# fpthink/EPC-Net

Hardware: AMD Instinct MI355X
Metric: point-clouds/sec (4096 pts) descriptor extraction (higher is better)
Workload: dtype f16x3; 1 GPU; epc-net inference, batch 64x4096x3 fp32 per GPU, NetVLAD K=64, 256-D output (BASELINE.json configs[1]); num_points=4096, precision=EPC_PRECISION_F32 (include/epcnet.h), weights=seeded random init of the architecture (no checkpoint payloads exist), parallelism=independent clouds sharded over 1 GPU(s), no data-path collective

## Files before the change

### epc-net_amd/csrc/head.hip

```cpp
#include "common.h"



template <int GROUPS>
__global__ __launch_bounds__(256) void vlad_fold_kernel(const float* __restrict__ V, const float* __restrict__ colss,
                                                        float* __restrict__ U) {
    constexpr int FPG = 1024 / GROUPS;
    __shared__ float cn[64];
    __shared__ float gsum[64];
    const int slab = blockIdx.x, cloud = blockIdx.y;
    const int k = threadIdx.x & 63, r = threadIdx.x >> 6;
    if (r == 0) {
        float t = 0.f;
#pragma unroll
        for (int g = 0; g < 32; ++g) t += colss[((size_t)cloud * 32 + g) * 64 + k];
        const float inv = 1.0f / sqrtf(fmaxf(t, 1e-12f));
        cn[k] = inv;
        gsum[k] = t * inv * inv;
    }
    __syncthreads();
    float tot = 0.f;
#pragma unroll
    for (int q = 0; q < 64; ++q) tot += gsum[q];
    const float sc = cn[k] * (1.0f / sqrtf(fmaxf(tot, 1e-12f)));
    const float* v = V + (size_t)cloud * 1024 * 64;
    float* uo = U + (size_t)cloud * FPG * 64;
#pragma unroll
    for (int m = 0; m < 4; ++m) {
        const int fi = 16 * slab + r + 4 * m;
        float u = 0.f;
#pragma unroll
        for (int g = 0; g < GROUPS; ++g) u += v[(size_t)(g * FPG + fi) * 64 + k] * sc;
        uo[(size_t)fi * 64 + k] = u;
    }
}

#define HSL 128
__global__ __launch_bounds__(64) void hidden_gemm_kernel(const float* __restrict__ U, const float* __restrict__ H,
                                                         int rows, int kh, float* __restrict__ Yp) {
    const int lane = threadIdx.x, j = lane & 31, h = lane >> 5;
    const int nb = blockIdx.x * 32;
    const int slice = blockIdx.y;
    const int m0 = blockIdx.z * 64;
    const int k0 = slice * HSL;
    f32x16 acc[2];
#pragma unroll
    for (int r = 0; r < 16; ++r) acc[0][r] = acc[1][r] = 0.f;
    const int r0 = m0 + j, r1 = m0 + 32 + j;
    const float* a0p = U + (size_t)min(r0, rows - 1) * kh + k0 + 4 * h;
    const float* a1p = U + (size_t)min(r1, rows - 1) * kh + k0 + 4 * h;
    const float z0 = r0 < rows ? 1.f : 0.f, z1 = r1 < rows ? 1.f : 0.f;
    const float* bp = H + (size_t)(k0 + 4 * h) * 256 + nb + j;
#pragma unroll 8
    for (int q = 0; q < HSL / 8; ++q) {
        const float4 a0 = *reinterpret_cast<const float4*>(a0p + 8 * q);
        const float4 a1 = *reinterpret_cast<const float4*>(a1p + 8 * q);
        const float b0 = bp[(size_t)(8 * q + 0) * 256], b1 = bp[(size_t)(8 * q + 1) * 256];
        const float b2 = bp[(size_t)(8 * q + 2) * 256], b3 = bp[(size_t)(8 * q + 3) * 256];
        acc[0] = mfma32(a0.x * z0, b0, acc[0]);
        acc[1] = mfma32(a1.x * z1, b0, acc[1]);
        acc[0] = mfma32(a0.y * z0, b1, acc[0]);
        acc[1] = mfma32(a1.y * z1, b1, acc[1]);
        acc[0] = mfma32(a0.z * z0, b2, acc[0]);
        acc[1] = mfma32(a1.z * z1, b2, acc[1]);
        acc[0] = mfma32(a0.w * z0, b3, acc[0]);
        acc[1] = mfma32(a1.w * z1, b3, acc[1]);
    }
#pragma unroll
    for (int t = 0; t < 2; ++t)
#pragma unroll
        for (int r = 0; r < 16; ++r) {
            const int row = m0 + 32 * t + mfma_row(r, h);
            if (row < rows) Yp[((size_t)slice * rows + row) * 256 + nb + j] = acc[t][r];
        }
}

__global__ __launch_bounds__(1024) void head_finish_kernel(const float* __restrict__ Yp, int slices, int rows,
                                                           const float* __restrict__ hp, int groups,
                                                           const int32_t* __restrict__ status,
                                                           float* __restrict__ out) {
    __shared__ float part_y[4][256];
    __shared__ float v[256];
    __shared__ float red[4];
    const int cloud = blockIdx.x, c = threadIdx.x & 255, part = threadIdx.x >> 8;
    const float* bn_s = hp;
    const float* bn_t = hp + 256;
    const float* Wg = hp + 512;
    const float* g_s = Wg + 65536;
    const float* g_t = g_s + 256;
    float y = 0.f;
    int s = part;
    for (; s + 28 < slices; s += 32) {
        float t[8];
#pragma unroll
        for (int u = 0; u < 8; ++u) t[u] = Yp[((size_t)(s + 4 * u) * rows + cloud) * 256 + c];
#pragma unroll
        for (int u = 0; u < 8; ++u) y += t[u];
    }
    for (; s < slices; s += 4) y += Yp[((size_t)s * rows + cloud) * 256 + c];
    part_y[part][c] = y;
    __syncthreads();
    const float val = ((part_y[0][c] + part_y[1][c]) + (part_y[2][c] + part_y[3][c])) * bn_s[c] + (float)groups * bn_t[c];
    if (part == 0) v[c] = val;
    __syncthreads();
    float g = 0.f;
#pragma unroll 16
    for (int k = 64 * part; k < 64 * part + 64; ++k) g += v[k] * Wg[k * 256 + c];
    part_y[part][c] = g;
    __syncthreads();
    g = (part_y[0][c] + part_y[1][c]) + (part_y[2][c] + part_y[3][c]);
    g = g * g_s[c] + g_t[c];
    const float o = val * (1.0f / (1.0f + expf(-g)));
    float ss = o * o;
#pragma unroll
    for (int off = 32; off >= 1; off >>= 1) ss += __shfl_xor(ss, off);
    if (part == 0 && (c & 63) == 0) red[c >> 6] = ss;
    __syncthreads();
    const float tot = (red[0] + red[1]) + (red[2] + red[3]);
    const bool poisoned = status && status[cloud] != 0;
    if (part == 0) out[(size_t)cloud * 256 + c] = poisoned ? __int_as_float(0x7fc00000) : o * (1.0f / sqrtf(fmaxf(tot, 1e-12f)));
}

__global__ __launch_bounds__(1024) void fc_head_kernel(const float* __restrict__ pooled,
                                                       const float* __restrict__ pack,
                                                       const int32_t* __restrict__ status, float* __restrict__ out) {
    __shared__ float m[1024];
    __shared__ float part_y[4][256];
    __shared__ float red[4];
    const int cloud = blockIdx.x, c = threadIdx.x & 255, part = threadIdx.x >> 8;
    m[threadIdx.x] = pooled[(size_t)cloud * 1024 + threadIdx.x];
    __syncthreads();
    float y = 0.f;
#pragma unroll 16
    for (int k = 256 * part; k < 256 * part + 256; ++k) y += m[k] * pack[k * 256 + c];
    part_y[part][c] = y;
    __syncthreads();
    y = fmaxf(((part_y[0][c] + part_y[1][c]) + (part_y[2][c] + part_y[3][c])) + pack[1024 * 256 + c], 0.f);
    float ss = y * y;
#pragma unroll
    for (int off = 32; off >= 1; off >>= 1) ss += __shfl_xor(ss, off);
    if (part == 0 && (c & 63) == 0) red[c >> 6] = ss;
    __syncthreads();
    const float tot = (red[0] + red[1]) + (red[2] + red[3]);
    const bool poisoned = status && status[cloud] != 0;
    if (part == 0) out[(size_t)cloud * 256 + c] = poisoned ? __int_as_float(0x7fc00000) : y * (1.0f / sqrtf(fmaxf(tot, 1e-12f)));
}

static inline size_t align_up(size_t v, size_t a) { return (v + a - 1) / a * a; }

extern "C" size_t epc_vlad_head_workspace_bytes(int num_clouds, int groups) {
    if (num_clouds <= 0 || groups <= 0 || 64 % groups) return 0;
    const size_t kh = 65536 / groups;
    const size_t u = align_up((size_t)num_clouds * kh * sizeof(float), 256);
    const size_t yp = align_up((kh / HSL) * (size_t)num_clouds * 256 * sizeof(float), 256);
    return u + yp;
}

extern "C" int epc_vlad_head_fwd(const float* V, const float* colss, const void* packed_head, int groups,
                                 int num_clouds, float* out, const int32_t* status, void* workspace,
                                 size_t workspace_bytes, void* stream) {
    EPC_CHECK_ARG(V && colss && packed_head && out && workspace, "null pointer");
    EPC_CHECK_ARG(groups > 0 && 64 % groups == 0, "GROUPS must divide 64");
    EPC_CHECK_ARG(num_clouds >= 0, "bad shape");
    if (num_clouds == 0) return EPC_OK;
    if (workspace_bytes < epc_vlad_head_workspace_bytes(num_clouds, groups)) {
        epc_set_error("epc_vlad_head_fwd: workspace too small");
        return EPC_ENOMEM;
    }
    const int kh = 65536 / groups;
    const float* hp = (const float*)packed_head;
    const float* Hw = hp + 65536;
    const float* tail = Hw + (size_t)kh * 256;
    char* wsp = (char*)workspace;
    float* U = (float*)wsp;
    wsp += align_up((size_t)num_clouds * kh * sizeof(float), 256);
    float* Yp = (float*)wsp;
    hipStream_t st = (hipStream_t)stream;
    EPC_CHECK_ARG(num_clouds <= 65535, "too many clouds per call");
    switch (groups) {
#define EPC_VF(G)                                                                                                  \
    case G:                                                                                                        \
        hipLaunchKernelGGL(vlad_fold_kernel<G>, dim3(1024 / G / 16, num_clouds), dim3(256), 0, st, V, colss, U);   \
        break;
        EPC_VF(1) EPC_VF(2) EPC_VF(4) EPC_VF(8) EPC_VF(16)
#undef EPC_VF
        default:
            epc_set_error("epc_vlad_head_fwd: GROUPS must be one of 1,2,4,8,16");
            return EPC_EINVAL;
    }
    EPC_CHECK_LAUNCH();
    const int slices = kh / HSL;
    hipLaunchKernelGGL(hidden_gemm_kernel, dim3(8, slices, (num_clouds + 63) / 64), dim3(64), 0, st, U, Hw,
                       num_clouds, kh, Yp);
    EPC_CHECK_LAUNCH();
    hipLaunchKernelGGL(head_finish_kernel, dim3(num_clouds), dim3(1024), 0, st, Yp, slices, num_clouds, tail,
                       groups, status, out);
    EPC_CHECK_LAUNCH();
    return EPC_OK;
}

extern "C" int epc_fc_head_fwd(const float* pooled, const void* packed_fc, int num_clouds, float* out,
                               const int32_t* status, void* stream) {
    EPC_CHECK_ARG(pooled && packed_fc && out, "null pointer");
    EPC_CHECK_ARG(num_clouds >= 0, "bad shape");
    if (num_clouds == 0) return EPC_OK;
    hipLaunchKernelGGL(fc_head_kernel, dim3(num_clouds), dim3(1024), 0, (hipStream_t)stream, pooled,
                       (const float*)packed_fc, status, out);
    EPC_CHECK_LAUNCH();
    return EPC_OK;
}
```

Measured before the change: 58410 clouds/s.

## Fuse VLAD group fold into hidden GEMM via LDS staging

Splits the per-cloud normalization scale into a small kernel and folds the group-sum of V directly into the hidden projection GEMM, staging the folded A tile in shared memory instead of writing and re-reading a U buffer in global memory. The GEMM now uses 256-thread blocks with 4 waves sharing an A tile, B values preloaded into registers, and A loads prefetched for small GROUPS. The finish kernel also preloads gate weights into registers and unrolls the slice reduction more deeply. This removes a global round trip of the large intermediate, at the cost of higher register pressure and possible occupancy loss.

```diff
diff --git a/epc-net_amd/csrc/head.hip b/epc-net_amd/csrc/head.hip
--- a/epc-net_amd/csrc/head.hip
+++ b/epc-net_amd/csrc/head.hip
@@ -2,69 +2,111 @@
 
 
 
+__global__ __launch_bounds__(64) void vlad_scale_kernel(const float* __restrict__ colss, float* __restrict__ sc) {
+    __shared__ float gsum[64];
+    const int cloud = blockIdx.x, k = threadIdx.x;
+    float t = 0.f;
+#pragma unroll
+    for (int g = 0; g < 32; ++g) t += colss[((size_t)cloud * 32 + g) * 64 + k];
+    const float inv = 1.0f / sqrtf(fmaxf(t, 1e-12f));
+    gsum[k] = t * inv * inv;
+    __syncthreads();
+    float tot = 0.f;
+#pragma unroll
+    for (int q = 0; q < 64; ++q) tot += gsum[q];
+    sc[(size_t)cloud * 64 + k] = inv * (1.0f / sqrtf(fmaxf(tot, 1e-12f)));
+}
+
+#define HSL 128
+#define HP_AROW (HSL + 4)
 template <int GROUPS>
-__global__ __launch_bounds__(256) void vlad_fold_kernel(const float* __restrict__ V, const float* __restrict__ colss,
-                                                        float* __restrict__ U) {
-    constexpr int FPG = 1024 / GROUPS;
-    __shared__ float cn[64];
-    __shared__ float gsum[64];
-    const int slab = blockIdx.x, cloud = blockIdx.y;
-    const int k = threadIdx.x & 63, r = threadIdx.x >> 6;
-    if (r == 0) {
-        float t = 0.f;
-#pragma unroll
-        for (int g = 0; g < 32; ++g) t += colss[((size_t)cloud * 32 + g) * 64 + k];
-        const float inv = 1.0f / sqrtf(fmaxf(t, 1e-12f));
-        cn[k] = inv;
-        gsum[k] = t * inv * inv;
-    }
-    __syncthreads();
-    float tot = 0.f;
-#pragma unroll
-    for (int q = 0; q < 64; ++q) tot += gsum[q];
-    const float sc = cn[k] * (1.0f / sqrtf(fmaxf(tot, 1e-12f)));
-    const float* v = V + (size_t)cloud * 1024 * 64;
-    float* uo = U + (size_t)cloud * FPG * 64;
-#pragma unroll
-    for (int m = 0; m < 4; ++m) {
-        const int fi = 16 * slab + r + 4 * m;
-        float u = 0.f;
-#pragma unroll
-        for (int g = 0; g < GROUPS; ++g) u += v[(size_t)(g * FPG + fi) * 64 + k] * sc;
-        uo[(size_t)fi * 64 + k] = u;
-    }
-}
-
-#define HSL 128
-__global__ __launch_bounds__(64) void hidden_gemm_kernel(const float* __restrict__ U, const float* __restrict__ H,
-                                                         int rows, int kh, float* __restrict__ Yp) {
-    const int lane = threadIdx.x, j = lane & 31, h = lane >> 5;
-    const int nb = blockIdx.x * 32;
-    const int slice = blockIdx.y;
-    const int m0 = blockIdx.z * 64;
+__global__ __launch_bounds__(256) void hidden_proj_kernel(const float* __restrict__ V, const float* __restrict__ sc,
+                                                          const float* __restrict__ H, int rows, float* __restrict__ Yp) {
+    constexpr int KH = 65536 / GROUPS;
+    constexpr bool PRE = GROUPS <= 4;
+    __shared__ __attribute__((aligned(16))) float As[64 * HP_AROW];
+    const int tid = threadIdx.x, lane = tid & 63, wave = tid >> 6, j = lane & 31, h = lane >> 5;
+    const int xi = blockIdx.x >> 3;
+    const int nb = (xi & 1) * 128 + wave * 32;
+    const int slice = (xi >> 1) * 8 + (blockIdx.x & 7);
+    const int m0 = blockIdx.y * 64;
     const int k0 = slice * HSL;
+    const float* bp = H + (size_t)(k0 + 4 * h) * 256 + nb + j;
+    float b[HSL / 8][4];
+    auto load_b = [&](int half) {
+#pragma unroll
+        for (int q = 8 * half; q < 8 * half + 8; ++q)
+#pragma unroll
+            for (int c = 0; c < 4; ++c) b[q][c] = bp[(size_t)(8 * q + c) * 256];
+    };
+    const int c4 = tid & 15, r0 = tid >> 4;
+    const float* vp[4];
+    float4 s4[4];
+    auto load_a = [&](int kb, int i, float4 (&v)[GROUPS]) {
+#pragma unroll
+        for (int g = 0; g < GROUPS; ++g) v[g] = *reinterpret_cast<const float4*>(vp[i] + (size_t)g * KH + 64 * kb);
+    };
+    auto fold_a = [&](int kb, int i, const float4 (&v)[GROUPS]) {
+        float4 u = make_float4(0.f, 0.f, 0.f, 0.f);
+#pragma unroll
+        for (int g = 0; g < GROUPS; ++g) {
+            u.x += v[g].x * s4[i].x;
+            u.y += v[g].y * s4[i].y;
+            u.z += v[g].z * s4[i].z;
+            u.w += v[g].w * s4[i].w;
+        }
+        *reinterpret_cast<float4*>(As + (r0 + 16 * i) * HP_AROW + 64 * kb + 4 * c4) = u;
+    };
     f32x16 acc[2];
 #pragma unroll
     for (int r = 0; r < 16; ++r) acc[0][r] = acc[1][r] = 0.f;
-    const int r0 = m0 + j, r1 = m0 + 32 + j;
-    const float* a0p = U + (size_t)min(r0, rows - 1) * kh + k0 + 4 * h;
-    const float* a1p = U + (size_t)min(r1, rows - 1) * kh + k0 + 4 * h;
-    const float z0 = r0 < rows ? 1.f : 0.f, z1 = r1 < rows ? 1.f : 0.f;
-    const float* bp = H + (size_t)(k0 + 4 * h) * 256 + nb + j;
-#pragma unroll 8
-    for (int q = 0; q < HSL / 8; ++q) {
-        const float4 a0 = *reinterpret_cast<const float4*>(a0p + 8 * q);
-        const float4 a1 = *reinterpret_cast<const float4*>(a1p + 8 * q);
-        const float b0 = bp[(size_t)(8 * q + 0) * 256], b1 = bp[(size_t)(8 * q + 1) * 256];
-        const float b2 = bp[(size_t)(8 * q + 2) * 256], b3 = bp[(size_t)(8 * q + 3) * 256];
-        acc[0] = mfma32(a0.x * z0, b0, acc[0]);
-        acc[1] = mfma32(a1.x * z1, b0, acc[1]);
-        acc[0] = mfma32(a0.y * z0, b1, acc[0]);
-        acc[1] = mfma32(a1.y * z1, b1, acc[1]);
-        acc[0] = mfma32(a0.z * z0, b2, acc[0]);
-        acc[1] = mfma32(a1.z * z1, b2, acc[1]);
-        acc[0] = mfma32(a0.w * z0, b3, acc[0]);
-        acc[1] = mfma32(a1.w * z1, b3, acc[1]);
+    const float* a0p = As + j * HP_AROW + 4 * h;
+    const float* a1p = As + (32 + j) * HP_AROW + 4 * h;
+    auto multiply = [&](int half) {
+#pragma unroll
+        for (int q = 8 * half; q < 8 * half + 8; ++q) {
+            const float4 a0 = *reinterpret_cast<const float4*>(a0p + 8 * q);
+            const float4 a1 = *reinterpret_cast<const float4*>(a1p + 8 * q);
+            acc[0] = mfma32(a0.x, b[q][0], acc[0]);
+            acc[1] = mfma32(a1.x, b[q][0], acc[1]);
+            acc[0] = mfma32(a0.y, b[q][1], acc[0]);
+            acc[1] = mfma32(a1.y, b[q][1], acc[1]);
+            acc[0] = mfma32(a0.z, b[q][2], acc[0]);
+            acc[1] = mfma32(a1.z, b[q][2], acc[1]);
+            acc[0] = mfma32(a0.w, b[q][3], acc[0]);
+            acc[1] = mfma32(a1.w, b[q][3], acc[1]);
+        }
+    };
+    float4 va[PRE ? 2 : 1][PRE ? 4 : 1][GROUPS];
+#pragma unroll
+    for (int i = 0; i < 4; ++i) {
+        const int row = min(m0 + r0 + 16 * i, rows - 1);
+        vp[i] = V + (size_t)row * 65536 + k0 + 4 * c4;
+        s4[i] = *reinterpret_cast<const float4*>(sc + (size_t)row * 64 + 4 * c4);
+    }
+    load_b(0);
+    if constexpr (PRE) {
+#pragma unroll
+        for (int i = 0; i < 4; ++i) load_a(0, i, va[0][i]);
+        load_b(1);
+#pragma unroll
+        for (int i = 0; i < 4; ++i) load_a(1, i, va[1][i]);
+    } else {
+        load_b(1);
+    }
+#pragma unroll
+    for (int kb = 0; kb < 2; ++kb) {
+#pragma unroll
+        for (int i = 0; i < 4; ++i) {
+            if constexpr (PRE) {
+                fold_a(kb, i, va[kb][i]);
+            } else {
+                load_a(kb, i, va[0][0]);
+                fold_a(kb, i, va[0][0]);
+            }
+        }
+        __syncthreads();
+        multiply(kb);
     }
 #pragma unroll
     for (int t = 0; t < 2; ++t)
@@ -88,8 +130,18 @@
     const float* Wg = hp + 512;
     const float* g_s = Wg + 65536;
     const float* g_t = g_s + 256;
+    float wg[64];
+#pragma unroll
+    for (int k = 0; k < 64; ++k) wg[k] = Wg[(64 * part + k) * 256 + c];
     float y = 0.f;
     int s = part;
+    for (; s + 124 < slices; s += 128) {
+        float t[32];
+#pragma unroll
+        for (int u = 0; u < 32; ++u) t[u] = Yp[((size_t)(s + 4 * u) * rows + cloud) * 256 + c];
+#pragma unroll
+        for (int u = 0; u < 32; ++u) y += t[u];
+    }
     for (; s + 28 < slices; s += 32) {
         float t[8];
 #pragma unroll
@@ -104,8 +156,8 @@
     if (part == 0) v[c] = val;
     __syncthreads();
     float g = 0.f;
-#pragma unroll 16
-    for (int k = 64 * part; k < 64 * part + 64; ++k) g += v[k] * Wg[k * 256 + c];
+#pragma unroll
+    for (int k = 0; k < 64; ++k) g += v[64 * part + k] * wg[k];
     part_y[part][c] = g;
     __syncthreads();
     g = (part_y[0][c] + part_y[1][c]) + (part_y[2][c] + part_y[3][c]);
@@ -151,7 +203,7 @@
 extern "C" size_t epc_vlad_head_workspace_bytes(int num_clouds, int groups) {
     if (num_clouds <= 0 || groups <= 0 || 64 % groups) return 0;
     const size_t kh = 65536 / groups;
-    const size_t u = align_up((size_t)num_clouds * kh * sizeof(float), 256);
+    const size_t u = align_up((size_t)num_clouds * 64 * sizeof(float), 256);
     const size_t yp = align_up((kh / HSL) * (size_t)num_clouds * 256 * sizeof(float), 256);
     return u + yp;
 }
@@ -172,26 +224,24 @@
     const float* Hw = hp + 65536;
     const float* tail = Hw + (size_t)kh * 256;
     char* wsp = (char*)workspace;
-    float* U = (float*)wsp;
-    wsp += align_up((size_t)num_clouds * kh * sizeof(float), 256);
+    float* sc = (float*)wsp;
+    wsp += align_up((size_t)num_clouds * 64 * sizeof(float), 256);
     float* Yp = (float*)wsp;
     hipStream_t st = (hipStream_t)stream;
     EPC_CHECK_ARG(num_clouds <= 65535, "too many clouds per call");
+    EPC_CHECK_ARG(groups == 1 || groups == 2 || groups == 4 || groups == 8 || groups == 16, "GROUPS must be one of 1,2,4,8,16");
+    hipLaunchKernelGGL(vlad_scale_kernel, dim3(num_clouds), dim3(64), 0, st, colss, sc);
+    EPC_CHECK_LAUNCH();
+    const int slices = kh / HSL;
+    const dim3 grid(2 * slices, (num_clouds + 63) / 64);
     switch (groups) {
-#define EPC_VF(G)                                                                                                  \
+#define EPC_HP(G)                                                                                                  \
     case G:                                                                                                        \
-        hipLaunchKernelGGL(vlad_fold_kernel<G>, dim3(1024 / G / 16, num_clouds), dim3(256), 0, st, V, colss, U);   \
+        hipLaunchKernelGGL(hidden_proj_kernel<G>, grid, dim3(256), 0, st, V, sc, Hw, num_clouds, Yp);              \
         break;
-        EPC_VF(1) EPC_VF(2) EPC_VF(4) EPC_VF(8) EPC_VF(16)
-#undef EPC_VF
-        default:
-            epc_set_error("epc_vlad_head_fwd: GROUPS must be one of 1,2,4,8,16");
-            return EPC_EINVAL;
-    }
-    EPC_CHECK_LAUNCH();
-    const int slices = kh / HSL;
-    hipLaunchKernelGGL(hidden_gemm_kernel, dim3(8, slices, (num_clouds + 63) / 64), dim3(64), 0, st, U, Hw,
-                       num_clouds, kh, Yp);
+        EPC_HP(1) EPC_HP(2) EPC_HP(4) EPC_HP(8) EPC_HP(16)
+#undef EPC_HP
+    }
     EPC_CHECK_LAUNCH();
     hipLaunchKernelGGL(head_finish_kernel, dim3(num_clouds), dim3(1024), 0, st, Yp, slices, num_clouds, tail,
                        groups, status, out);
```

Result: no change. 58710 clouds/s, median of 6 (+0.5%).
